# CogSP/CoEvoNet

Measured on AMD Instinct MI355X. Metric: env-steps/sec (agent-steps of the whole job; generations/sec in gens_per_sec), Co-GA simple_adversary_v3 pop=200 HoF=5, higher is better.
Workload: dtype f32

## Files before the change

### coevonet_amd/build.py

```python
import os
import subprocess
import sys
from concurrent.futures import ThreadPoolExecutor

HERE = os.path.dirname(os.path.abspath(__file__))
CSRC = os.path.join(HERE, "csrc")
OBJ = os.path.join(HERE, "csrc", "_obj")
LIB = os.path.join(HERE, "libcoevo.so")
SOURCES = ["fc_forward.hip", "mpe_env.hip", "offspring.hip", "select.hip", "rollout_api.hip", "deepqn.hip",
           "dqn_engine.hip", "host_rollout.hip", "host_placement.hip", "fc16.hip", "fc16_rollout.hip", "fc16_offspring.hip",
           "fc16_es.hip", "dqn16.hip", "dqn16_offspring.hip", "dqn16_es.hip", "dqn16_tiled.hip", "crossplay.hip",
           "sharing.hip"]
FLAGS = ["--offload-arch=gfx950", "-O3", "-std=c++17", "-fPIC", "-ffp-contract=off", "-fno-fast-math", "-Wall",
         "-Wno-unused-function"]


def _headers():
    hs = [os.path.join(CSRC, f) for f in os.listdir(CSRC) if f.endswith(".h")]
    return hs + [os.path.join(HERE, "..", "include", h) for h in ("coevo.h", "coevo_ext.h", "coevo_crossplay.h",
                                                                   "coevo_sharing.h")]


def _stale(target, deps):
    if not os.path.exists(target):
        return True
    t = os.path.getmtime(target)
    return any(os.path.getmtime(d) > t for d in deps)


def _extra_flags():
    return os.environ.get("COEVO_EXTRA_FLAGS", "").split()


def _flag_signature():
    return " ".join(FLAGS + _extra_flags())
# ... 46 lines not shown
```

### coevonet_amd/csrc/mpe_env.hip

```cpp
#include "coevo_common.hip.h"

#include "../../include/coevo_crossplay.h"

namespace coevo {

typedef unsigned __int128 u128;

__host__ __device__ inline u128 pcg_mult()
{
    return (((u128)0x2360ED051FC65DA4ULL) << 64) | (u128)0x4385DF649FCCF645ULL;
}

__host__ __device__ inline uint64_t pcg_output(u128 s)
{
    const uint64_t hi = (uint64_t)(s >> 64), lo = (uint64_t)s;
    const uint64_t x = hi ^ lo;
    const unsigned r = (unsigned)(hi >> 58);
    return (x >> r) | (x << ((64 - r) & 63));
}

__host__ __device__ inline u128 pcg_advance(u128 state, u128 inc, u128 delta)
{
    u128 acc_mult = 1, acc_plus = 0, cur_mult = pcg_mult(), cur_plus = inc;
    while (delta > 0) {
        if (delta & 1) {
            acc_mult *= cur_mult;
            acc_plus = acc_plus * cur_mult + cur_plus;
        }
        cur_plus = (cur_mult + 1) * cur_plus;
        cur_mult *= cur_mult;
        delta >>= 1;
    }
    return acc_mult * state + acc_plus;
}

__host__ __device__ __forceinline__ void mpe_reset_game(double *st, int n, int g, coevo_pcg64 rng, uint64_t ordinal);

__global__ void mpe_reset_kernel(double *st, int n, int game_first, int count, coevo_pcg64 rng,
                                 int64_t first_ordinal, const int32_t *gen_dev, int64_t ordinals_per_gen, int unsigned_first)
{
    const int i = blockIdx.x * blockDim.x + threadIdx.x;
    if (i >= count) return;
    int64_t first = first_ordinal + (gen_dev ? (int64_t)(*gen_dev) * ordinals_per_gen : 0);
    if (first < 0 && !unsigned_first) first = 0;
    mpe_reset_game(st, n, game_first + i, rng, (uint64_t)first + (uint64_t)i);
}

__global__ void mpe_reset_episodes_kernel(double *st, int n, int game_first, int count, coevo_pcg64 rng,
                                          uint64_t first_ordinal, int episodes)
{
    const int i = blockIdx.x * blockDim.x + threadIdx.x;
// ... 5 lines not shown
struct ResetSegs { coevo_reset_seg s[COEVO_MAX_JOBS]; };
__global__ void mpe_reset_multi_kernel(double *st, int n, ResetSegs segs, coevo_pcg64 rng, uint64_t *stamps, int n_stamps,
                                       int32_t *zero_words, int n_zero)
{
    const coevo_reset_seg &sg = segs.s[blockIdx.y];
    const int i = blockIdx.x * blockDim.x + threadIdx.x;
    if (zero_words && blockIdx.y == gridDim.y - 1)
        for (int j = i; j < n_zero; j += gridDim.x * blockDim.x) zero_words[j] = 0;
    if (stamps && blockIdx.y == 0)
        for (int j = i; j < n_stamps; j += gridDim.x * blockDim.x) {
            stamps[2 * j] = ~0ull;
            stamps[2 * j + 1] = 0ull;
        }
    if (i >= sg.count) return;
    mpe_reset_game(st, n, sg.game_first + i, rng, sg.first_ordinal + (uint64_t)i);
}

__host__ __device__ __forceinline__ void mpe_reset_game(double *st, int n, int g, coevo_pcg64 rng, uint64_t ordinal)
{
    const u128 inc = ((u128)rng.pcg_inc_hi << 64) | rng.pcg_inc_lo;
    u128 s = ((u128)rng.pcg_state_hi << 64) | rng.pcg_state_lo;
    s = pcg_advance(s, inc, (u128)(ordinal >> 1) * 21);
    s = s * pcg_mult() + inc;
    const uint64_t c = pcg_output(s);
    const uint32_t half = (ordinal & 1) ? (uint32_t)(c >> 32) : (uint32_t)c;
    const int goal = (int)(((uint64_t)half * 2) >> 32);
    if (ordinal & 1) s = pcg_advance(s, inc, 10);
    double d[10];
#pragma unroll
    for (int i = 0; i < 10; ++i) {
        s = s * pcg_mult() + inc;
        d[i] = -1.0 + 2.0 * ((double)(pcg_output(s) >> 11) * (1.0 / 9007199254740992.0));
    }
    const size_t N = (size_t)n;
#pragma unroll
    for (int i = 0; i < 6; ++i) {
        st[i * N + g] = d[i];
        st[(6 + i) * N + g] = 0.0;
    }
#pragma unroll
    for (int i = 0; i < 4; ++i) st[(12 + i) * N + g] = d[6 + i];
    st[16 * N + g] = d[6 + 2 * goal];
    st[17 * N + g] = d[7 + 2 * goal];
    st[18 * N + g] = 0.0;
    st[19 * N + g] = 0.0;
    st[20 * N + g] = 0.0;
    st[21 * N + g] = 0.0;
    st[22 * N + g] = (double)goal;
    st[23 * N + g] = 0.0;
}

__host__ __device__ inline float mpe_observe_at(const double *st, int n, const int32_t *row_game, const int32_t *row_slot, int i)
{
    const int row = i / COEVO_OBS_STRIDE, k = i % COEVO_OBS_STRIDE;
    const int slot = row_slot[row];
    const int D = (slot == COEVO_SLOT_ADVERSARY) ? 8 : 10;
    return (k < D) ? mpe_obs_element(st, n, row_game[row], slot, k) : 0.0f;
}

__global__ void mpe_observe_kernel(const double *st, int n, const int32_t *row_game, const int32_t *row_slot,
                                   int n_rows, float *obs)
{
    const int i = blockIdx.x * blockDim.x + threadIdx.x;
    if (i >= n_rows * COEVO_OBS_STRIDE) return;
// ... 358 lines not shown
```

### coevonet_amd/csrc/offspring.hip

```cpp
#include "coevo_common.hip.h"
#include "dqn_common.hip.h"
#include "promote_roles.hip.h"
#include "philox.hip.h"

namespace coevo {

__device__ __forceinline__ uint32_t w2_piece_quad(int32_t s0, int32_t o_w2)
{
    const int32_t t = s0 - o_w2;
    const int32_t l = (t >> 2) & 63, kq = (t >> 8) & 127, jb = t >> 15;
    return (uint32_t)((o_w2 + (jb * 64 + l) * H1 + kq * 4) >> 2);
}

__device__ __forceinline__ int32_t w1t_slab_of_flat(uint32_t p, int D)
{
    const uint32_t j = (D == 8) ? (p >> 3) : (p / 10u);
    return (int32_t)((p - j * (uint32_t)D) * H1 + j);
}

__device__ inline void slab_quad_normals(uint64_t seed, uint32_t slo, uint32_t shi, int32_t s0, int D, float z[4])
{
    const int32_t o_b1 = (int32_t)fc_off_b1(D), o_w2 = (int32_t)fc_off_w2(D), o_b2 = (int32_t)fc_off_b2(D);
    const int32_t P = (int32_t)fc_params(D);
    if (s0 >= o_w2 && s0 < o_b2) {
// ... 85 lines not shown
    v = v + dpp_move_f64<0x4E>(v);
    v = v + dpp_move_f64<0x141>(v);
    v = v + dpp_move_f64<0x140>(v);
    v = add_swap_f64<false>(v);
    v = add_swap_f64<true>(v);
    if ((threadIdx.x & 63) == 0) scratch[threadIdx.x >> 6] = v;
    __syncthreads();
    return ((scratch[0] + scratch[1]) + scratch[2]) + scratch[3];
}

#ifndef COEVO_BREED_U
#define COEVO_BREED_U 2
#endif

struct alignas(16) PerturbLds { float z[W1T_MAX_FLOATS]; };

__device__ __forceinline__ void fc_perturb_block(const float *parent_slab, const int32_t *parent_idx, float *child_slab,
                                                 int child_first, int D, const float *sigma_dev, uint64_t seed,
                                                 uint32_t stream_lo_first, uint32_t stream_hi, int skip_layernorm,
                                                 const int32_t *gen_dev, const float *dist_ref, double *dist_partial,
                                                 int c, int bx, int nblocks, PerturbLds &lds)
{
    const int w1t_blocks = D / 2;
    if (bx > 0 && bx < w1t_blocks) return;
    if (gen_dev) stream_hi += 4u * (uint32_t)(*gen_dev);
    const bool antithetic = (skip_layernorm & 2) != 0;
    skip_layernorm &= 1;
    const uint32_t ind = stream_lo_first + (uint32_t)c;
    const uint32_t slo = antithetic ? (ind >> 1) : ind;
    const bool negate = antithetic && (ind & 1u);
// ... 4 lines not shown
    double *scratch = reinterpret_cast<double *>(lds.z);
    if (bx == 0) {
        w1t_normals_to_lds(seed, slo, stream_hi, D, lds.z);
        const float4 *zl = reinterpret_cast<const float4 *>(lds.z);
        float4 zv = zl[threadIdx.x];
        __syncthreads();
        const bool keep[4] = {false, false, false, false}, in_dist[4] = {true, true, true, true};
        for (int b = 0; b < w1t_blocks; ++b) {
            const int32_t s0 = (b * 256 + (int32_t)threadIdx.x) * 4;
            const float4 pv = *reinterpret_cast<const float4 *>(par + s0);
            const float z[4] = {zv.x, zv.y, zv.z, zv.w};
            const double d2 = perturb_apply_piece(pv, z, keep, in_dist, sigma, negate, ch, dist_ref, s0);
            if (b + 1 < w1t_blocks) zv = zl[(b + 1) * 256 + threadIdx.x];
            if (dist_partial) {
                const double tot = breed_block_sum(d2, scratch + 4 * (b & 1));
                if (threadIdx.x == 0) dist_partial[(size_t)c * nblocks + b] = tot;
            }
        }
        return;
    }
#if COEVO_BREED_U > 1
    {
        const int32_t o_w2 = (int32_t)fc_off_w2(D), o_b2 = (int32_t)fc_off_b2(D);
        const int w2_first = (o_w2 + 1023) >> 10, w2_end = o_b2 >> 10;
        if (bx >= w2_first && bx < w2_end) {
            if ((bx - w2_first) % COEVO_BREED_U) return;
            const int run = min(COEVO_BREED_U, w2_end - bx);
            const bool keep[4] = {false, false, false, false}, in_dist[4] = {true, true, true, true};
            double d2u[COEVO_BREED_U];
#pragma unroll
            for (int u = 0; u < COEVO_BREED_U; ++u) {
                d2u[u] = 0.0;
                if (u < run) {
                    const int32_t s0 = ((bx + u) * 256 + (int32_t)threadIdx.x) * 4;
                    const float4 pv = *reinterpret_cast<const float4 *>(par + s0);
                    float z[4];
                    philox_normal4(seed, slo, stream_hi, w2_piece_quad(s0, o_w2), z);
                    d2u[u] = perturb_apply_piece(pv, z, keep, in_dist, sigma, negate, ch, dist_ref, s0);
                }
            }
            if (dist_partial) {
#pragma unroll
                for (int u = 0; u < COEVO_BREED_U; ++u) {
                    if (u < run) {
                        const double tot = breed_block_sum(d2u[u], scratch + 4 * (u & 1));
                        if (threadIdx.x == 0) dist_partial[(size_t)c * nblocks + bx + u] = tot;
                    }
                }
            }
            return;
        }
    }
#endif
    const int32_t s0 = (bx * 256 + (int32_t)threadIdx.x) * 4;
    double d2 = 0.0;
    if (s0 < (int32_t)stride) {
        const float4 pv = *reinterpret_cast<const float4 *>(par + s0);
        float z[4];
        bool keep[4], in_dist[4];
        const int32_t o_w2 = (int32_t)fc_off_w2(D), o_b2 = (int32_t)fc_off_b2(D);
        if (s0 >= o_w2 && s0 < o_b2) {
// ... 3 lines not shown
        } else {
            slab_quad_normals(seed, slo, stream_hi, s0, D, z);
            const int32_t g1 = (int32_t)fc_off_g1(D), g2 = (int32_t)fc_off_g2(D), P = (int32_t)fc_params(D);
            const bool ln = (s0 >= g1 && s0 < g1 + 2 * H1) || (s0 >= g2 && s0 < g2 + 2 * H2);
#pragma unroll
            for (int i = 0; i < 4; ++i) {
                const bool pad = s0 + i >= P;
                keep[i] = pad || (skip_layernorm && ln);
                in_dist[i] = !pad && !ln;
            }
        }
        d2 = perturb_apply_piece(pv, z, keep, in_dist, sigma, negate, ch, dist_ref, s0);
    }
    if (dist_partial) {
        const double tot = breed_block_sum(d2, scratch);
        if (threadIdx.x == 0) dist_partial[(size_t)c * nblocks + bx] = tot;
    }
}

__global__ __launch_bounds__(256) void fc_perturb_kernel(const float *parent_slab, const int32_t *parent_idx,
                                                          float *child_slab, int child_first, int D,
                                                          const float *sigma_dev, uint64_t seed,
                                                          uint32_t stream_lo_first, uint32_t stream_hi,
                                                          int skip_layernorm, const int32_t *gen_dev,
                                                          const float *dist_ref, double *dist_partial)
{
    __shared__ PerturbLds lds;
    fc_perturb_block(parent_slab, parent_idx, child_slab, child_first, D, sigma_dev, seed, stream_lo_first, stream_hi,
                     skip_layernorm, gen_dev, dist_ref, dist_partial, blockIdx.y, blockIdx.x, gridDim.x, lds);
}

static_assert(sizeof(coevo_fc_perturb_job) == 72, "layout mirrored by coevonet_amd/lib.py PerturbJob");
struct PerturbJobs { coevo_fc_perturb_job j[COEVO_MAX_JOBS]; };
__global__ __launch_bounds__(256) void fc_perturb_multi_kernel(PerturbJobs jobs, uint64_t seed, int skip_layernorm,
                                                                const int32_t *gen_dev)
{
    __shared__ PerturbLds lds;
    const coevo_fc_perturb_job &jb = jobs.j[blockIdx.z];
    const int nblocks = (int)quad_blocks(fc_stride(jb.D));
    if ((int)blockIdx.x >= nblocks || (int)blockIdx.y >= jb.n_children) return;
    fc_perturb_block(jb.parent_slab, jb.parent_idx, jb.child_slab, jb.child_first, jb.D, jb.sigma_dev, seed,
                     jb.stream_lo_first, jb.stream_hi, skip_layernorm, gen_dev, jb.dist_ref, jb.dist_partial, blockIdx.y,
                     blockIdx.x, nblocks, lds);
}

__global__ __launch_bounds__(256) void fc_rebuild_elites_kernel(const float *elite_prev, const int32_t *order,
                                                                 float *elite_new, int E, int D,
                                                                 const float *sigma_prev_dev, uint64_t seed,
                                                                 uint32_t stream_hi_prev, const int32_t *gen_dev)
{
    if (gen_dev) stream_hi_prev += 4u * (uint32_t)(*gen_dev - 1);
    const int e = blockIdx.y;
    const int64_t stride = fc_stride(D), P = fc_params(D);
    const int64_t s0 = quad_first(blockIdx.x);
    if (s0 >= stride) return;
    const int id = order[e];
    float *dst = elite_new + (int64_t)e * stride;
    if (id == 0) {
// ... 356 lines not shown
    for (int i = 0; i < n_jobs; ++i) {
        const coevo_fc_perturb_job &j = jobs[i];
        if (!perturb_job_ok(j)) return COEVO_ERR_ARG;
        pj.j[i] = j;
        const unsigned nb = quad_blocks(fc_stride(j.D));
        gx = nb > gx ? nb : gx;
        gy = (unsigned)j.n_children > gy ? (unsigned)j.n_children : gy;
    }
    if (gy == 0) return COEVO_OK;
    hipLaunchKernelGGL(fc_perturb_multi_kernel, dim3(gx, gy, (unsigned)n_jobs), dim3(256), 0, (hipStream_t)stream, pj, seed,
                       skip_layernorm, gen_dev);
    COEVO_HIP_CHECK(hipGetLastError());
    return COEVO_OK;
}

extern "C" int coevo_fc_rebuild_elites(const float *elite_prev, const int32_t *order, float *elite_new, int E, int D,
                                       const float *sigma_prev_dev, uint64_t seed, uint32_t stream_hi_prev,
                                       const int32_t *gen_dev, void *stream)
{
    if (!elite_prev || !order || !elite_new || !sigma_prev_dev || !fc_dim_ok(D) || E <= 0 || E > 65535)
        return COEVO_ERR_ARG;
    if (elite_prev == elite_new) return COEVO_ERR_ARG;
    const dim3 grid(quad_blocks(fc_stride(D)), (unsigned)E);
    hipLaunchKernelGGL(fc_rebuild_elites_kernel, grid, dim3(256), 0, (hipStream_t)stream, elite_prev, order, elite_new,
                       E, D, sigma_prev_dev, seed, stream_hi_prev, gen_dev);
    COEVO_HIP_CHECK(hipGetLastError());
    return COEVO_OK;
}

extern "C" int coevo_net_gather(const float *src_slab, const int32_t *src_idx, float *dst_slab, int dst_first, int n,
// ... 208 lines not shown
```

### coevonet_amd/genetic_algorithm.py

```python
from __future__ import annotations

import os
import time

import numpy as np
import torch

from . import lib as L
from .fcnetwork import FCNetwork
from .ga_half import HalfGAEngine
from .game_logic import create_agent
from .mpe.simple_adversary import ENV_SEED
from .population import (FUSED_MAX_HOF, GA_SHARING_MODES, N_EVAL, RET_SLOT, ROLE_D, ROLES, SIGMA_ATTR, CoGASchedule, CoGATail,
                         NetTable, SlabIO, adapt_mutation_power, captured, co_ga_games, eval_gate_limits, fused_tail_fits,
                         half_route, mean_eval_triple, shard_and_gather, slab_layout)
from .rollout import DeviceRollout, HostEnvRollout, RolloutPlan, effective_steps

ROLE_SLOT = {"agent_0": 1, "agent_1": 2, "adversary_0": 0}


def evaluate_current_weights(agent_0, agent_1, adversary, env, args):
    from .game_logic import play_game
    tot = [0.0, 0.0, 0.0]
    for _ in range(N_EVAL):
        r = play_game(env=env, player1=agent_0.model, player2=agent_1.model, adversary=adversary.model, args=args, eval=True)
        for s in range(3):
            tot[s] += r[s]
    return tot[0] / 10, tot[1] / 10, tot[2] / 10


def mutate_elites(env, elites, args, role):
# ... 163 lines not shown
            self.pair_scratch = torch.zeros(n_scratch, dtype=torch.float64, device=device)
        self.parent_idx = torch.tensor([c % elites for c in range(max(pop - 1, 1))], dtype=torch.int32, device=device)
        self.hof_shift_idx = torch.arange(1, max(hof, 2), dtype=torch.int32, device=device)
        self.iota = torch.arange(max(hof, elites, 2), dtype=torch.int32, device=device)
        self.pblocks = {r: int(L.load().coevo_fc_perturb_blocks(ROLE_D[r])) for r in ROLES}
        self.dist_partial = {r: torch.zeros(max(pop - 1, 1) * self.pblocks[r], dtype=torch.float64, device=device) for r in ROLES}
        self.best_dist = {r: torch.zeros(1, **f32) for r in ROLES}
        one = torch.arange(self.n_local, device=device) * hof + hof - 1
        self._last_game_idx = torch.cat([ph * self.n_local * hof + one for ph in range(3)])
        self.generation = 0
        self.steps_per_generation = 3 * pop * hof * self.T_train + N_EVAL * self.T_eval
        self._dist_current = False
        self._rewards_pin = self._rewards_dev = None
        self._breeding_pending, self.generation_enqueued = False, 0
        self._cohort_streams = self._cohort_done = self._tail_done = self._tail_graph = None
        self.sharded_run, self._sharded_tail_graphs = False, {}
        self.gen_dev = self.sigma64 = self.sigma32 = self.sigma32_prev = self.hist = self.sig_hist = self.loop_args = None
        self.cap, self.fused_tail, self.pipelined, self._gen_graph = 0, False, False, {}

    def _need_device_loop(self):
        if self.gen_dev is None:
            raise RuntimeError("GAEngine: setup_device_loop(args, capacity) has to be called before a device-loop generation")

    def _uploaded(self, region):
        if region in ("pop", "stale"):
            self._dist_current = False
        if region == "hof" and self._hof_tiled:
            self._refresh_hof_twins()

    def _refresh_hof_twins(self):
# ... 193 lines not shown
    def _breed_cohort(self, k, noise_gen, gen_dev=None, tick=False):
        lo_k, hi_k = self._cohort_individuals(k)
        c_lo, c_hi = max(lo_k, 1) - 1, hi_k - 1
        if c_hi > c_lo:
            sigma, stream = self.sigma32.data_ptr(), 0 if gen_dev is not None else noise_gen * 4
            self._breed_children_multi(c_lo, c_hi, (sigma, sigma + 4, sigma + 8), (stream, stream + 1, stream + 2), gen_dev,
                                       L._p(self.gen_dev) if tick else None)
            return
        if lo_k == 0:
            for r in ROLES:
                self.dist[r][0:1].copy_(self.best_dist[r])
        if tick:
            L.call("coevo_counter_add", L._p(self.gen_dev), 1)

    def _reset_cohort(self, k, gen):
        segs = self._reset_segments(gen, *self._cohort_individuals(k), k == self.K - 1 and gen > 0)
        self.ro.reset_segments(segs, arm=(k, self.n_cycles))

    def flush_breeding(self):
        if self._breeding_pending:
            torch.cuda.synchronize()
            for k in range(self.K):
                self._breed_cohort(k, self.generation_enqueued - 1)
            torch.cuda.synchronize()
            self._breeding_pending = False

    def replay_generation_pipelined(self, gen):
        self._need_device_loop()
        assert self.world == 1 and self.env_mode == "device" and self.fused_tail and self.K > 1
        if self.hof_twin is not None and not self._hof_tiled and self.plan.heavy is not None:
            self._enable_hof_tiled()
        self._enqueue_cohort_chains(gen)
# ... 6 lines not shown
    def _enqueue_cohort_chains(self, gen):
        ro = self.ro
        self._gate_evaluation(gen)
        main = torch.cuda.current_stream()
        if self._cohort_streams is None:
            self._cohort_streams = [main] + [
                torch.cuda.ExternalStream(L.load().coevo_rollout_ctx_cohort_stream(ro.ctx, k), device=self.device)
                for k in range(1, self.K)]
            self._cohort_done = [torch.cuda.Event() for _ in range(self.K)]
            self._tail_done = torch.cuda.Event()
        self._tail_done.record(main)
        for k, s in reversed(list(enumerate(self._cohort_streams))):
            if k:
                s.wait_event(self._tail_done)
            with torch.cuda.stream(s):
                if self._breeding_pending:
                    self._breed_cohort(k, gen - 1)
                self._reset_cohort(k, gen)
                ro.enqueue_cohort(k, self.n_cycles, s, armed=True)
            if k:
                self._cohort_done[k].record(s)
        self._breeding_pending = False
        for ev in self._cohort_done[1:]:
            main.wait_event(ev)
        ro.enqueue_final_step(self.n_cycles, pack=self._pack_args() if self._packed_exchange() else None)

    def _packed_exchange(self):
        return (self.sharded_run and self.fused_tail and self.gather_packed is not None
                and os.environ.get("COEVO_PACKED_EXCHANGE", "1") != "0")

    def _pack_args(self):
        return (self.pack_local, self.dist_all, 3, self.n_local, self.hof, self.pop, self.lo)

# ... 330 lines not shown
```

### coevonet_amd/lib.py

```python
from __future__ import annotations

import ctypes as C
import math
import os
import re

import numpy as np
import torch

HERE = os.path.dirname(os.path.abspath(__file__))
LIB_PATH = os.environ.get("COEVO_LIB") or os.path.join(HERE, "libcoevo.so")
HEADER_PATH = os.path.join(HERE, "..", "include", "coevo.h")
EXT_HEADER_PATH = os.path.join(HERE, "..", "include", "coevo_ext.h")
CROSSPLAY_HEADER_PATH = os.path.join(HERE, "..", "include", "coevo_crossplay.h")
SHARING_HEADER_PATH = os.path.join(HERE, "..", "include", "coevo_sharing.h")


class CoevoError(RuntimeError):
    pass


_SCALARS = {"int": C.c_int, "int32_t": C.c_int32, "int64_t": C.c_int64, "uint32_t": C.c_uint32, "uint64_t": C.c_uint64,
            "size_t": C.c_size_t, "float": C.c_float, "double": C.c_double}
_POINTED_TO = ("void", "char", "uint8_t")


def _declare(text, structs, decl, spec=None):
    m = re.fullmatch(r"([\w\s]*?)\s*(\**)\s*(\w+)\s*(?:\[(\d+)\])?", text.strip())
    words = [w for w in (m.group(1).split() if m else []) if w not in ("const", "struct")]
    if not m or len(words) > 1 or not (words or spec):
# ... 103 lines not shown

K_XP, _XP_SIGS = _parse_crossplay_header(_header_text(CROSSPLAY_HEADER_PATH))


def _parse_sharing_header(text):
    consts, structs, sigs = parse_header(text, known=STRUCTS)
    if (set(structs) != set(STRUCTS) or set(sigs) & (set(_SIGS) | set(_EXT_SIGS) | set(_XP_SIGS))
            or set(consts) & (set(K) | set(K_EXT) | set(K_XP))):
        raise CoevoError("include/coevo_sharing.h: declares a struct or repeats a name of include/coevo.h, include/coevo_ext.h "
                         "or include/coevo_crossplay.h")
    return consts, sigs


K_SH, _SH_SIGS = _parse_sharing_header(_header_text(SHARING_HEADER_PATH))

OBS_STRIDE, LOGIT_STRIDE, FC_MAX_ROWS = K["COEVO_OBS_STRIDE"], K["COEVO_LOGIT_STRIDE"], K["COEVO_FC_MAX_ROWS"]
MPE_STATE_DOUBLES, STAMP_SLOTS = K["COEVO_MPE_STATE_DOUBLES"], K["COEVO_STAMP_SLOTS"]
ST_NAMES = {K["COEVO_ST_BAD_INPUT"]: "input contains inf or NaN",
            K["COEVO_ST_BAD_FC1"]: "output contains inf or NaN after fc1",
            K["COEVO_ST_BAD_FC2"]: "output contains inf or NaN after fc2",
            K["COEVO_ST_BAD_OUT"]: "output contains inf or NaN",
            K["COEVO_ST_NO_ACTION"]: "no action selected (current_best_position = -1)",
            K["COEVO_ST_SYNC_TIMEOUT"]: "persistent rollout: a workgroup timed out waiting for the other rows of its games "
                                        "(COEVO_ST_SYNC_TIMEOUT)",
            K["COEVO_ST_BAD_TASK"]: "fp16 forward: a task with a bad width, row count or unaligned net offset was skipped "
                                    "(COEVO_ST_BAD_TASK)"}

DQN_LOGIT_STRIDE, DQN_MAX_ROWS = K["COEVO_DQN_LOGIT_STRIDE"], K["COEVO_DQN_MAX_ROWS"]
DQN_FC1_TILED = K["COEVO_DQN_FC1_TILED"]
DQP_SKIP_BN = K["COEVO_DQP_SKIP_BN"]
# ... 31 lines not shown
    return sorted(_SIGS)


def extension_symbols():
    return sorted(_EXT_SIGS)


def crossplay_symbols():
    return sorted(_XP_SIGS)


def sharing_symbols():
    return sorted(_SH_SIGS)


def load():
    global _lib
    if _lib is None:
        if not os.path.exists(LIB_PATH):
            raise CoevoError(f"{LIB_PATH} is missing: build the HIP extension first "
                             "(python -m coevonet_amd.build); there is no CPU fallback")
        L = C.CDLL(LIB_PATH)
        for name, (res, args) in {**_SIGS, **_EXT_SIGS, **_XP_SIGS, **_SH_SIGS}.items():
            fn = getattr(L, name)
            fn.restype = res
            fn.argtypes = args
        flags = (L.coevo_build_flags() or b"").decode()
        if flags and os.environ.get("COEVO_ALLOW_VARIANT") != "1":
            raise CoevoError(f"{LIB_PATH} was built with non-default switches ({flags}): a measurement variant, not the "
                             "product (rebuild with python -m coevonet_amd.build, or set COEVO_ALLOW_VARIANT=1 in tools/)")
        _lib = L
    return _lib


def _check(rc, what):
    if rc != 0:
        raise CoevoError(f"{what} failed with code {rc} "
                         f"({'bad argument' if rc == -1 else 'HIP runtime error' if rc == -2 else 'unsupported here' if rc == -3 else 'unknown'})")
# ... 70 lines not shown
```

### coevonet_amd/population.py

```python
from __future__ import annotations

import ctypes as ct
import os

import numpy as np
import torch

from . import lib as L
from .rollout import DeviceRollout, RolloutPlan

ROLES = ("agent_0", "agent_1", "adversary_0")
ROLE_D = {"agent_0": 10, "agent_1": 10, "adversary_0": 8}
RET_SLOT = {"agent_0": 0, "agent_1": 1, "adversary_0": 2}
ROLES2 = ("first_0", "second_0")
N_EVAL = 10
ES_CHUNKS = 8
SIGMA_ATTR = {"agent_0": "mutation_power_agent_0", "agent_1": "mutation_power_agent_1",
              "adversary_0": "mutation_power_adversary"}


def slab_layout(roles, regions, stride_of):
    base, off = {}, 0
    for r in roles:
        base[r] = {}
# ... 300 lines not shown

    def _promote_unfused(self, r, best_to_pop0=True, best_dist=False):
        self._hof_push(r)
        if best_to_pop0:
            self._best_to_pop0(r)
        if best_dist:
            L.call("coevo_gather_f32", L._p(self.best_dist[r]), L._p(self.dist[r]), L._p(self.order[r]), 1)

    def _breed_role_children(self, ri, r, c_lo, c_hi, stream, gen_dev, sigma_ptr):
        L.call(self._perturb_dist_entry, self._ptr(r, "elite"), self.parent_idx.data_ptr() + 4 * c_lo, self._ptr(r, "pop"),
               1 + c_lo, c_hi - c_lo, ROLE_D[r], sigma_ptr, self.philox_seed, c_lo, stream, 0, gen_dev, self._ptr(r, "stale"),
               L._p(self.dist_partial[r]))
        L.call(self._finalize_entry, L._p(self.dist_partial[r]), self.pblocks[r], c_hi - c_lo, L._p(self.dist[r]), 1 + c_lo,
               L._p(self.best_dist[r]) if c_lo == 0 else None)

    def _breed_children_multi(self, c_lo, c_hi, sigma_ptrs, streams, gen_dev=None, tick=None):
        Job = getattr(L, self._perturb_job)
        pj, fj = (Job * 3)(), (L.FinalizeJob * 3)()
        for ri, r in enumerate(ROLES):
            part = self.dist_partial[r].data_ptr() + 8 * c_lo * self.pblocks[r]
            pj[ri] = Job(self._ptr(r, "elite"), self.parent_idx.data_ptr() + 4 * c_lo, self._ptr(r, "pop"), sigma_ptrs[ri],
                         self._ptr(r, "stale"), part, 1 + c_lo, c_hi - c_lo, ROLE_D[r], c_lo, streams[ri], 0)
            fj[ri] = L.FinalizeJob(part, self.dist[r].data_ptr(), self.best_dist[r].data_ptr() if c_lo == 0 else None,
                                   self.pblocks[r], c_hi - c_lo, 1 + c_lo, 0)
        L.call(self._perturb_multi_entry, ct.cast(pj, ct.c_void_p), 3, self.philox_seed, 0, gen_dev)
        if tick is not None:
            L.call(self._finalize_multi_entry + "_tick", ct.cast(fj, ct.c_void_p), 3, tick)
        else:
            L.call(self._finalize_multi_entry, ct.cast(fj, ct.c_void_p), 3)


class CoESSchedule:

    def _rollout_pair(self, games, eval_games, table, env_seed, cls=DeviceRollout, host_cohorts=None, **ro_kw):
        cohorts = int(os.environ.get("COEVO_ES_COHORTS", "2")) if host_cohorts is None else host_cohorts
        game_cohort = None
        if host_cohorts is not None and cohorts > 1 and len(games) >= cohorts:
            game_cohort = (np.arange(len(games)) * cohorts // len(games)).astype(np.int32)
        self.plan = RolloutPlan(np.array(games), table.net_off, table.net_D, device=self.device,
# ... 169 lines not shown
```

### coevonet_amd/rollout.py

```python
from __future__ import annotations

import ctypes as _ct

import os

import numpy as np
import torch

from . import lib as L
from .mpe import simple_adversary as sa

LIGHT_ROWS = 8
HEAVY_ROWS = 32


class RolloutPlan:

    def __init__(self, game_nets, net_off, net_D, device="cuda", heavy_rows=HEAVY_ROWS, n_cohorts=1,
                 game_cohort=None, split_rows=None, row_order="class", resident_nets=()):
        game_nets = np.asarray(game_nets, dtype=np.int64)
        self.n_games = int(game_nets.shape[0])
        by_net = {}
        for g in range(self.n_games):
            for slot in range(3):
# ... 122 lines not shown

    def cohort_tasks(self, k):
        out = ()
        for tasks, tnp, begin in ((self.heavy, self.heavy_np, self.heavy_begin_np), (self.light, self.light_np, self.light_begin_np)):
            b, e = int(begin[k]), int(begin[k + 1])
            ptr = tasks.data_ptr() + b * L.TASK_DTYPE.itemsize if (tasks is not None and e > b) else None
            out += (ptr, e - b, int(max(tnp["n_rows"][b:e], default=0)))
        return out

    def distinct_weight_bytes_per_cycle(self):
        seen = {}
        for arr in (self.heavy_np, self.light_np):
            for t in arr:
                seen[int(t["net_off"])] = L.fc_param_count(int(t["D"])) * 4
        return sum(seen.values())


def effective_steps(limit, max_cycles):
    cap = 3 * max_cycles
    return cap if limit is None else min(int(limit), cap)


def last_buffer(n_cycles):
    last = int(n_cycles) - 1
    return last & 1 if last > 0 else 0


class DeviceRollout:

    def __init__(self, plan: RolloutPlan, slab: torch.Tensor, env_seed=sa.ENV_SEED, timing_pairs=0, fused_step=True,
# ... 65 lines not shown
        try:
            if getattr(self, "ctx", None):
                L.load().coevo_rollout_ctx_destroy(self.ctx)
                self.ctx = None
        except Exception:
            pass

    def set_limits(self, limits_np):
        self.limits.copy_(torch.from_numpy(np.asarray(limits_np, dtype=np.int32)), non_blocking=False)

    def reset(self, game_first, n_games, first_ordinal):
        L.call("coevo_mpe_reset", L._p(self.state), self.plan.n_games, int(game_first), int(n_games), self.rng,
               int(first_ordinal))

    def reset_segments(self, segs, arm=None):
        arr = (L.ResetSeg * len(segs))(*[L.ResetSeg(int(a), int(b), int(c)) for a, b, c in segs])
        if arm is not None:
            k, n_cycles = arm
            n_cycles = int(n_cycles)
            if k is not None and not 0 <= int(k) < self.n_cohorts:
                raise ValueError(f"arm: cohort {k} of a rollout with {self.n_cohorts}")
            if not 0 < n_cycles <= self.stamp_cycles:
                raise ValueError(f"arm: {n_cycles} cycles (1 .. {self.stamp_cycles})")
            first, count = (0, self.n_cohorts) if k is None else (int(k), 1)
            stamps, sync = self._cohort_scratch(first, n_cycles)
            if stamps or sync:
                L.call("coevo_mpe_reset_multi_prep", L._p(self.state), self.plan.n_games, _ct.cast(arr, _ct.c_void_p), len(segs),
                       self.rng, stamps, count * n_cycles * L.STAMP_SLOTS if stamps else 0, sync,
                       count * self.sync_words_per_cohort if sync else 0)
            else:
                L.call("coevo_mpe_reset_multi", L._p(self.state), self.plan.n_games, _ct.cast(arr, _ct.c_void_p), len(segs),
                       self.rng)
            for c in range(first, first + count):
                self._armed[c] = (n_cycles, bool(self.time_light))
            return
        L.call("coevo_mpe_reset_multi", L._p(self.state), self.plan.n_games, _ct.cast(arr, _ct.c_void_p), len(segs), self.rng)

    def _take_arm(self, cohorts, n_cycles, armed):
        if armed:
            for c in cohorts:
                if self._armed.get(c) != (int(n_cycles), bool(self.time_light)):
                    raise ValueError(f"armed=True, but cohort {c} was not armed for {n_cycles} cycles"
                                     f"{' with timed stamps' if self.time_light else ''} by reset_segments(arm=...) since its "
                                     f"last rollout (armed: {self._armed})")
        for c in cohorts:
            self._armed.pop(c, None)

    def _cohort_scratch(self, k, n_cycles):
        stamps = (self.stamps.data_ptr() + 16 * L.STAMP_SLOTS * int(k) * int(n_cycles)) if self.time_light else None
        sync = (self.sync_words.data_ptr() + 4 * int(k) * self.sync_words_per_cohort) if self.sync_words is not None else None
        return stamps, sync
# ... 262 lines not shown
```

Before: 153.8 million.

## Fuse per-cohort breeding, distance finalize and env reset into one turnover kernel

Adds a ga_turnover_kernel that, in a single launch, runs the per-cohort episode resets, stamp and sync-word clears, the perturbation of the children and their distance partials. The last workgroup for each child is detected with an atomic ticket counter and reduces the distance partials in place. In the pipelined Co-GA loop, the separate perturb, finalize and reset launches per cohort are replaced by this one call, which cuts launch count and host overhead per cohort. In exchange it uses atomic ticket counters with relaxed ordering and a waitcnt, so correctness depends on memory visibility between workgroups, and the reset blocks now share a grid with the heavier perturb blocks.

```diff
diff --git a/coevonet_amd/build.py b/coevonet_amd/build.py
--- a/coevonet_amd/build.py
+++ b/coevonet_amd/build.py
@@ -18,7 +18,7 @@
 def _headers():
     hs = [os.path.join(CSRC, f) for f in os.listdir(CSRC) if f.endswith(".h")]
     return hs + [os.path.join(HERE, "..", "include", h) for h in ("coevo.h", "coevo_ext.h", "coevo_crossplay.h",
-                                                                   "coevo_sharing.h")]
+                                                                   "coevo_sharing.h", "coevo_turnover.h")]
 
 
 def _stale(target, deps):
diff --git a/coevonet_amd/csrc/mpe_env.hip b/coevonet_amd/csrc/mpe_env.hip
--- a/coevonet_amd/csrc/mpe_env.hip
+++ b/coevonet_amd/csrc/mpe_env.hip
@@ -1,40 +1,10 @@
 #include "coevo_common.hip.h"
+#include "mpe_reset.hip.h"
 
 #include "../../include/coevo_crossplay.h"
 
 namespace coevo {
 
-typedef unsigned __int128 u128;
-
-__host__ __device__ inline u128 pcg_mult()
-{
-    return (((u128)0x2360ED051FC65DA4ULL) << 64) | (u128)0x4385DF649FCCF645ULL;
-}
-
-__host__ __device__ inline uint64_t pcg_output(u128 s)
-{
-    const uint64_t hi = (uint64_t)(s >> 64), lo = (uint64_t)s;
-    const uint64_t x = hi ^ lo;
-    const unsigned r = (unsigned)(hi >> 58);
-    return (x >> r) | (x << ((64 - r) & 63));
-}
-
-__host__ __device__ inline u128 pcg_advance(u128 state, u128 inc, u128 delta)
-{
-    u128 acc_mult = 1, acc_plus = 0, cur_mult = pcg_mult(), cur_plus = inc;
-    while (delta > 0) {
-        if (delta & 1) {
-            acc_mult *= cur_mult;
-            acc_plus = acc_plus * cur_mult + cur_plus;
-        }
-        cur_plus = (cur_mult + 1) * cur_plus;
-        cur_mult *= cur_mult;
-        delta >>= 1;
-    }
-    return acc_mult * state + acc_plus;
-}
-
-__host__ __device__ __forceinline__ void mpe_reset_game(double *st, int n, int g, coevo_pcg64 rng, uint64_t ordinal);
 
 __global__ void mpe_reset_kernel(double *st, int n, int game_first, int count, coevo_pcg64 rng,
                                  int64_t first_ordinal, const int32_t *gen_dev, int64_t ordinals_per_gen, int unsigned_first)
@@ -70,40 +40,6 @@
         }
     if (i >= sg.count) return;
     mpe_reset_game(st, n, sg.game_first + i, rng, sg.first_ordinal + (uint64_t)i);
-}
-
-__host__ __device__ __forceinline__ void mpe_reset_game(double *st, int n, int g, coevo_pcg64 rng, uint64_t ordinal)
-{
-    const u128 inc = ((u128)rng.pcg_inc_hi << 64) | rng.pcg_inc_lo;
-    u128 s = ((u128)rng.pcg_state_hi << 64) | rng.pcg_state_lo;
-    s = pcg_advance(s, inc, (u128)(ordinal >> 1) * 21);
-    s = s * pcg_mult() + inc;
-    const uint64_t c = pcg_output(s);
-    const uint32_t half = (ordinal & 1) ? (uint32_t)(c >> 32) : (uint32_t)c;
-    const int goal = (int)(((uint64_t)half * 2) >> 32);
-    if (ordinal & 1) s = pcg_advance(s, inc, 10);
-    double d[10];
-#pragma unroll
-    for (int i = 0; i < 10; ++i) {
-        s = s * pcg_mult() + inc;
-        d[i] = -1.0 + 2.0 * ((double)(pcg_output(s) >> 11) * (1.0 / 9007199254740992.0));
-    }
-    const size_t N = (size_t)n;
-#pragma unroll
-    for (int i = 0; i < 6; ++i) {
-        st[i * N + g] = d[i];
-        st[(6 + i) * N + g] = 0.0;
-    }
-#pragma unroll
-    for (int i = 0; i < 4; ++i) st[(12 + i) * N + g] = d[6 + i];
-    st[16 * N + g] = d[6 + 2 * goal];
-    st[17 * N + g] = d[7 + 2 * goal];
-    st[18 * N + g] = 0.0;
-    st[19 * N + g] = 0.0;
-    st[20 * N + g] = 0.0;
-    st[21 * N + g] = 0.0;
-    st[22 * N + g] = (double)goal;
-    st[23 * N + g] = 0.0;
 }
 
 __host__ __device__ inline float mpe_observe_at(const double *st, int n, const int32_t *row_game, const int32_t *row_slot, int i)
diff --git a/coevonet_amd/csrc/mpe_reset.hip.h b/coevonet_amd/csrc/mpe_reset.hip.h
--- /dev/null
+++ b/coevonet_amd/csrc/mpe_reset.hip.h
@@ -0,0 +1,70 @@
+#pragma once
+#include "coevo_common.hip.h"
+
+namespace coevo {
+
+typedef unsigned __int128 u128;
+
+__host__ __device__ inline u128 pcg_mult()
+{
+    return (((u128)0x2360ED051FC65DA4ULL) << 64) | (u128)0x4385DF649FCCF645ULL;
+}
+
+__host__ __device__ inline uint64_t pcg_output(u128 s)
+{
+    const uint64_t hi = (uint64_t)(s >> 64), lo = (uint64_t)s;
+    const uint64_t x = hi ^ lo;
+    const unsigned r = (unsigned)(hi >> 58);
+    return (x >> r) | (x << ((64 - r) & 63));
+}
+
+__host__ __device__ inline u128 pcg_advance(u128 state, u128 inc, u128 delta)
+{
+    u128 acc_mult = 1, acc_plus = 0, cur_mult = pcg_mult(), cur_plus = inc;
+    while (delta > 0) {
+        if (delta & 1) {
+            acc_mult *= cur_mult;
+            acc_plus = acc_plus * cur_mult + cur_plus;
+        }
+        cur_plus = (cur_mult + 1) * cur_plus;
+        cur_mult *= cur_mult;
+        delta >>= 1;
+    }
+    return acc_mult * state + acc_plus;
+}
+
+__host__ __device__ __forceinline__ void mpe_reset_game(double *st, int n, int g, coevo_pcg64 rng, uint64_t ordinal)
+{
+    const u128 inc = ((u128)rng.pcg_inc_hi << 64) | rng.pcg_inc_lo;
+    u128 s = ((u128)rng.pcg_state_hi << 64) | rng.pcg_state_lo;
+    s = pcg_advance(s, inc, (u128)(ordinal >> 1) * 21);
+    s = s * pcg_mult() + inc;
+    const uint64_t c = pcg_output(s);
+    const uint32_t half = (ordinal & 1) ? (uint32_t)(c >> 32) : (uint32_t)c;
+    const int goal = (int)(((uint64_t)half * 2) >> 32);
+    if (ordinal & 1) s = pcg_advance(s, inc, 10);
+    double d[10];
+#pragma unroll
+    for (int i = 0; i < 10; ++i) {
+        s = s * pcg_mult() + inc;
+        d[i] = -1.0 + 2.0 * ((double)(pcg_output(s) >> 11) * (1.0 / 9007199254740992.0));
+    }
+    const size_t N = (size_t)n;
+#pragma unroll
+    for (int i = 0; i < 6; ++i) {
+        st[i * N + g] = d[i];
+        st[(6 + i) * N + g] = 0.0;
+    }
+#pragma unroll
+    for (int i = 0; i < 4; ++i) st[(12 + i) * N + g] = d[6 + i];
+    st[16 * N + g] = d[6 + 2 * goal];
+    st[17 * N + g] = d[7 + 2 * goal];
+    st[18 * N + g] = 0.0;
+    st[19 * N + g] = 0.0;
+    st[20 * N + g] = 0.0;
+    st[21 * N + g] = 0.0;
+    st[22 * N + g] = (double)goal;
+    st[23 * N + g] = 0.0;
+}
+
+}
diff --git a/coevonet_amd/csrc/offspring.hip b/coevonet_amd/csrc/offspring.hip
--- a/coevonet_amd/csrc/offspring.hip
+++ b/coevonet_amd/csrc/offspring.hip
@@ -2,6 +2,9 @@
 #include "dqn_common.hip.h"
 #include "promote_roles.hip.h"
 #include "philox.hip.h"
+#include "mpe_reset.hip.h"
+
+#include "../../include/coevo_turnover.h"
 
 namespace coevo {
 
@@ -123,6 +126,11 @@
 #endif
 
 struct alignas(16) PerturbLds { float z[W1T_MAX_FLOATS]; };
+
+__device__ __forceinline__ void store_partial(double *p, double v)
+{
+    __hip_atomic_store(p, v, __ATOMIC_RELAXED, __HIP_MEMORY_SCOPE_AGENT);
+}
 
 __device__ __forceinline__ void fc_perturb_block(const float *parent_slab, const int32_t *parent_idx, float *child_slab,
                                                  int child_first, int D, const float *sigma_dev, uint64_t seed,
@@ -157,7 +165,7 @@
             if (b + 1 < w1t_blocks) zv = zl[(b + 1) * 256 + threadIdx.x];
             if (dist_partial) {
                 const double tot = breed_block_sum(d2, scratch + 4 * (b & 1));
-                if (threadIdx.x == 0) dist_partial[(size_t)c * nblocks + b] = tot;
+                if (threadIdx.x == 0) store_partial(dist_partial + (size_t)c * nblocks + b, tot);
             }
         }
         return;
@@ -187,7 +195,7 @@
                 for (int u = 0; u < COEVO_BREED_U; ++u) {
                     if (u < run) {
                         const double tot = breed_block_sum(d2u[u], scratch + 4 * (u & 1));
-                        if (threadIdx.x == 0) dist_partial[(size_t)c * nblocks + bx + u] = tot;
+                        if (threadIdx.x == 0) store_partial(dist_partial + (size_t)c * nblocks + bx + u, tot);
                     }
                 }
             }
@@ -221,7 +229,7 @@
     }
     if (dist_partial) {
         const double tot = breed_block_sum(d2, scratch);
-        if (threadIdx.x == 0) dist_partial[(size_t)c * nblocks + bx] = tot;
+        if (threadIdx.x == 0) store_partial(dist_partial + (size_t)c * nblocks + bx, tot);
     }
 }
 
@@ -249,6 +257,65 @@
     fc_perturb_block(jb.parent_slab, jb.parent_idx, jb.child_slab, jb.child_first, jb.D, jb.sigma_dev, seed,
                      jb.stream_lo_first, jb.stream_hi, skip_layernorm, gen_dev, jb.dist_ref, jb.dist_partial, blockIdx.y,
                      blockIdx.x, nblocks, lds);
+}
+
+struct TurnoverJobs {
+    coevo_fc_perturb_job p[COEVO_MAX_JOBS];
+    coevo_fc_finalize_job f[COEVO_MAX_JOBS];
+    coevo_reset_seg s[COEVO_MAX_JOBS];
+};
+struct TurnoverGrid { uint32_t reset_wgs, rx, n_segs, gx, gy; };
+
+__global__ __launch_bounds__(256) void ga_turnover_kernel(TurnoverJobs tj, TurnoverGrid gd, uint64_t seed, int skip_layernorm,
+                                                          const int32_t *gen_dev, uint32_t *tickets, double *st, int n,
+                                                          coevo_pcg64 rng, uint64_t *stamps, int n_stamps, int32_t *zero_words,
+                                                          int n_zero)
+{
+    __shared__ PerturbLds lds;
+    uint32_t wg = blockIdx.x;
+    if (wg < gd.reset_wgs) {
+        const uint32_t sy = wg / gd.rx;
+        const int i = (int)((wg % gd.rx) * 256u + threadIdx.x), span = (int)(gd.rx * 256u);
+        if (zero_words && sy == gd.n_segs - 1)
+            for (int j = i; j < n_zero; j += span) zero_words[j] = 0;
+        if (stamps && sy == 0)
+            for (int j = i; j < n_stamps; j += span) {
+                stamps[2 * j] = ~0ull;
+                stamps[2 * j + 1] = 0ull;
+            }
+        const coevo_reset_seg &sg = tj.s[sy];
+        if (i < sg.count) mpe_reset_game(st, n, sg.game_first + i, rng, sg.first_ordinal + (uint64_t)i);
+        return;
+    }
+    wg -= gd.reset_wgs;
+    const uint32_t bx = wg % gd.gx, cy = wg / gd.gx, c = cy % gd.gy, job = cy / gd.gy;
+    const coevo_fc_perturb_job &jb = tj.p[job];
+    const int nblocks = (int)quad_blocks(fc_stride(jb.D));
+    if ((int)bx >= nblocks || (int)c >= jb.n_children) return;
+    fc_perturb_block(jb.parent_slab, jb.parent_idx, jb.child_slab, jb.child_first, jb.D, jb.sigma_dev, seed,
+                     jb.stream_lo_first, jb.stream_hi, skip_layernorm, gen_dev, jb.dist_ref, jb.dist_partial, (int)c, (int)bx,
+                     nblocks, lds);
+    __syncthreads();
+    int *last = reinterpret_cast<int *>(lds.z) + 16;
+    if (threadIdx.x == 0) {
+        uint32_t *t = tickets + (size_t)job * gd.gy + c;
+        __builtin_amdgcn_s_waitcnt(0);
+        const uint32_t before = __hip_atomic_fetch_add(t, 1u, __ATOMIC_RELAXED, __HIP_MEMORY_SCOPE_AGENT);
+        *last = before == (uint32_t)nblocks - 1u;
+        if (*last) __hip_atomic_store(t, 0u, __ATOMIC_RELAXED, __HIP_MEMORY_SCOPE_AGENT);
+    }
+    __syncthreads();
+    if (!*last || threadIdx.x >= 64) return;
+    const coevo_fc_finalize_job &fj = tj.f[job];
+    const double *pp = fj.dist_partial + (size_t)c * fj.n_blocks;
+    double v = 0.0;
+    for (int b = threadIdx.x; b < fj.n_blocks; b += 64) v += __hip_atomic_load(pp + b, __ATOMIC_RELAXED, __HIP_MEMORY_SCOPE_AGENT);
+#pragma unroll
+    for (int m = 1; m < 64; m <<= 1) v = v + __shfl_xor(v, m, 64);
+    if (threadIdx.x == 0) {
+        fj.dist[fj.first + (int)c] = (float)sqrt(v);
+        if (c == 0 && fj.head) fj.dist[fj.first - 1] = *fj.head;
+    }
 }
 
 __global__ __launch_bounds__(256) void fc_rebuild_elites_kernel(const float *elite_prev, const int32_t *order,
@@ -635,6 +702,50 @@
     return COEVO_OK;
 }
 
+extern "C" int coevo_ga_turnover(const coevo_fc_perturb_job *jobs, const coevo_fc_finalize_job *fin, int n_jobs, uint64_t seed,
+                                 int skip_layernorm, const int32_t *gen_dev, uint32_t *tickets, double *state, int n_games,
+                                 const coevo_reset_seg *segs, int n_segs, coevo_pcg64 rng, uint64_t *stamps, int n_stamps,
+                                 int32_t *zero_words, int n_zero, void *stream)
+{
+    if (!jobs || !fin || !tickets || n_jobs < 1 || n_jobs > COEVO_MAX_JOBS || skip_layernorm < 0 || skip_layernorm > 3)
+        return COEVO_ERR_ARG;
+    if (!state || n_games <= 0 || !segs || n_segs < 1 || n_segs > COEVO_MAX_JOBS) return COEVO_ERR_ARG;
+    if ((stamps && n_stamps <= 0) || (zero_words && n_zero <= 0)) return COEVO_ERR_ARG;
+    TurnoverJobs tj{};
+    uint32_t gx = 0, gy = 0;
+    for (int i = 0; i < n_jobs; ++i) {
+        const coevo_fc_perturb_job &j = jobs[i];
+        const coevo_fc_finalize_job &f = fin[i];
+        if (!perturb_job_ok(j) || !j.dist_partial) return COEVO_ERR_ARG;
+        const uint32_t nb = quad_blocks(fc_stride(j.D));
+        if (f.dist_partial != j.dist_partial || !f.dist || f.n_blocks != (int)nb || f.n != j.n_children || f.first < 0 ||
+            (f.head && f.first < 1))
+            return COEVO_ERR_ARG;
+        tj.p[i] = j;
+        tj.f[i] = f;
+        gx = nb > gx ? nb : gx;
+        gy = (uint32_t)j.n_children > gy ? (uint32_t)j.n_children : gy;
+    }
+    int cmax = 0;
+    for (int i = 0; i < n_segs; ++i) {
+        if (segs[i].game_first < 0 || segs[i].count < 0 || segs[i].game_first + segs[i].count > n_games) return COEVO_ERR_ARG;
+        tj.s[i] = segs[i];
+        cmax = segs[i].count > cmax ? segs[i].count : cmax;
+    }
+    if (!stamps) n_stamps = 0;
+    if (!zero_words) n_zero = 0;
+    const bool resets = cmax > 0 || stamps || zero_words;
+    const uint32_t rx = cmax > 0 ? (uint32_t)(cmax + 255) / 256u : 1u;
+    const TurnoverGrid gd{resets ? rx * (uint32_t)n_segs : 0u, rx, (uint32_t)n_segs, gx, gy};
+    const uint64_t total = (uint64_t)gd.reset_wgs + (uint64_t)gx * gy * (uint32_t)n_jobs;
+    if (total == 0) return COEVO_OK;
+    if (total > 0xffffffffull) return COEVO_ERR_ARG;
+    hipLaunchKernelGGL(ga_turnover_kernel, dim3((uint32_t)total), dim3(256), 0, (hipStream_t)stream, tj, gd, seed, skip_layernorm,
+                       gen_dev, tickets, state, n_games, rng, stamps, n_stamps, zero_words, n_zero);
+    COEVO_HIP_CHECK(hipGetLastError());
+    return COEVO_OK;
+}
+
 extern "C" int coevo_fc_rebuild_elites(const float *elite_prev, const int32_t *order, float *elite_new, int E, int D,
                                        const float *sigma_prev_dev, uint64_t seed, uint32_t stream_hi_prev,
                                        const int32_t *gen_dev, void *stream)
diff --git a/coevonet_amd/genetic_algorithm.py b/coevonet_amd/genetic_algorithm.py
--- a/coevonet_amd/genetic_algorithm.py
+++ b/coevonet_amd/genetic_algorithm.py
@@ -1,5 +1,6 @@
 from __future__ import annotations
 
+import ctypes as ct
 import os
 import time
 
@@ -14,7 +15,7 @@
 from .population import (FUSED_MAX_HOF, GA_SHARING_MODES, N_EVAL, RET_SLOT, ROLE_D, ROLES, SIGMA_ATTR, CoGASchedule, CoGATail,
                          NetTable, SlabIO, adapt_mutation_power, captured, co_ga_games, eval_gate_limits, fused_tail_fits,
                          half_route, mean_eval_triple, shard_and_gather, slab_layout)
-from .rollout import DeviceRollout, HostEnvRollout, RolloutPlan, effective_steps
+from .rollout import DeviceRollout, HostEnvRollout, RolloutPlan, effective_steps, reset_seg_array
 
 ROLE_SLOT = {"agent_0": 1, "agent_1": 2, "adversary_0": 0}
 
@@ -208,6 +209,7 @@
         self._rewards_pin = self._rewards_dev = None
         self._breeding_pending, self.generation_enqueued = False, 0
         self._cohort_streams = self._cohort_done = self._tail_done = self._tail_graph = None
+        self._turnover_tickets = None
         self.sharded_run, self._sharded_tail_graphs = False, {}
         self.gen_dev = self.sigma64 = self.sigma32 = self.sigma32_prev = self.hist = self.sig_hist = self.loop_args = None
         self.cap, self.fused_tail, self.pipelined, self._gen_graph = 0, False, False, {}
@@ -431,8 +433,34 @@
             L.call("coevo_counter_add", L._p(self.gen_dev), 1)
 
     def _reset_cohort(self, k, gen):
-        segs = self._reset_segments(gen, *self._cohort_individuals(k), k == self.K - 1 and gen > 0)
-        self.ro.reset_segments(segs, arm=(k, self.n_cycles))
+        self.ro.reset_segments(self._cohort_segments(k, gen), arm=(k, self.n_cycles))
+
+    def _cohort_segments(self, k, gen):
+        return self._reset_segments(gen, *self._cohort_individuals(k), k == self.K - 1 and gen > 0)
+
+    def _turnover_args(self, k, gen):
+        lo_k, hi_k = self._cohort_individuals(k)
+        c_lo, c_hi = max(lo_k, 1) - 1, hi_k - 1
+        if c_hi <= c_lo:
+            return None
+        sigma, stream = self.sigma32.data_ptr(), (gen - 1) * 4
+        pj, fj = self._multi_jobs(c_lo, c_hi, (sigma, sigma + 4, sigma + 8), (stream, stream + 1, stream + 2))
+        return pj, fj, self._cohort_segments(k, gen)
+
+    def _turnover_cohort(self, k, gen):
+        args = self._turnover_args(k, gen) if self._breeding_pending else None
+        if args is None:
+            if self._breeding_pending:
+                self._breed_cohort(k, gen - 1)
+            self._reset_cohort(k, gen)
+            return
+        pj, fj, segs = args
+        if self._turnover_tickets is None:
+            self._turnover_tickets = torch.zeros(self.K, 3 * max(self.pop, 1), dtype=torch.int32, device=self.device)
+        ro, arr = self.ro, reset_seg_array(segs)
+        L.call("coevo_ga_turnover", ct.cast(pj, ct.c_void_p), ct.cast(fj, ct.c_void_p), 3, self.philox_seed, 0, None,
+               self._turnover_tickets[k].data_ptr(), L._p(ro.state), self.plan.n_games, ct.cast(arr, ct.c_void_p), len(segs),
+               ro.rng, *ro.arm_scratch(k, self.n_cycles))
 
     def flush_breeding(self):
         if self._breeding_pending:
@@ -469,9 +497,7 @@
             if k:
                 s.wait_event(self._tail_done)
             with torch.cuda.stream(s):
-                if self._breeding_pending:
-                    self._breed_cohort(k, gen - 1)
-                self._reset_cohort(k, gen)
+                self._turnover_cohort(k, gen)
                 ro.enqueue_cohort(k, self.n_cycles, s, armed=True)
             if k:
                 self._cohort_done[k].record(s)
diff --git a/coevonet_amd/lib.py b/coevonet_amd/lib.py
--- a/coevonet_amd/lib.py
+++ b/coevonet_amd/lib.py
@@ -14,6 +14,7 @@
 EXT_HEADER_PATH = os.path.join(HERE, "..", "include", "coevo_ext.h")
 CROSSPLAY_HEADER_PATH = os.path.join(HERE, "..", "include", "coevo_crossplay.h")
 SHARING_HEADER_PATH = os.path.join(HERE, "..", "include", "coevo_sharing.h")
+TURNOVER_HEADER_PATH = os.path.join(HERE, "..", "include", "coevo_turnover.h")
 
 
 class CoevoError(RuntimeError):
@@ -147,6 +148,17 @@
 
 K_SH, _SH_SIGS = _parse_sharing_header(_header_text(SHARING_HEADER_PATH))
 
+
+def _parse_turnover_header(text):
+    consts, structs, sigs = parse_header(text, known=STRUCTS)
+    if (set(structs) != set(STRUCTS) or set(sigs) & (set(_SIGS) | set(_EXT_SIGS) | set(_XP_SIGS) | set(_SH_SIGS))
+            or set(consts) & (set(K) | set(K_EXT) | set(K_XP) | set(K_SH))):
+        raise CoevoError("include/coevo_turnover.h: declares a struct or repeats a name of another header")
+    return consts, sigs
+
+
+K_TO, _TO_SIGS = _parse_turnover_header(_header_text(TURNOVER_HEADER_PATH))
+
 OBS_STRIDE, LOGIT_STRIDE, FC_MAX_ROWS = K["COEVO_OBS_STRIDE"], K["COEVO_LOGIT_STRIDE"], K["COEVO_FC_MAX_ROWS"]
 MPE_STATE_DOUBLES, STAMP_SLOTS = K["COEVO_MPE_STATE_DOUBLES"], K["COEVO_STAMP_SLOTS"]
 ST_NAMES = {K["COEVO_ST_BAD_INPUT"]: "input contains inf or NaN",
@@ -208,6 +220,10 @@
     return sorted(_SH_SIGS)
 
 
+def turnover_symbols():
+    return sorted(_TO_SIGS)
+
+
 def load():
     global _lib
     if _lib is None:
@@ -215,7 +231,7 @@
             raise CoevoError(f"{LIB_PATH} is missing: build the HIP extension first "
                              "(python -m coevonet_amd.build); there is no CPU fallback")
         L = C.CDLL(LIB_PATH)
-        for name, (res, args) in {**_SIGS, **_EXT_SIGS, **_XP_SIGS, **_SH_SIGS}.items():
+        for name, (res, args) in {**_SIGS, **_EXT_SIGS, **_XP_SIGS, **_SH_SIGS, **_TO_SIGS}.items():
             fn = getattr(L, name)
             fn.restype = res
             fn.argtypes = args
diff --git a/coevonet_amd/population.py b/coevonet_amd/population.py
--- a/coevonet_amd/population.py
+++ b/coevonet_amd/population.py
@@ -338,7 +338,7 @@
         L.call(self._finalize_entry, L._p(self.dist_partial[r]), self.pblocks[r], c_hi - c_lo, L._p(self.dist[r]), 1 + c_lo,
                L._p(self.best_dist[r]) if c_lo == 0 else None)
 
-    def _breed_children_multi(self, c_lo, c_hi, sigma_ptrs, streams, gen_dev=None, tick=None):
+    def _multi_jobs(self, c_lo, c_hi, sigma_ptrs, streams):
         Job = getattr(L, self._perturb_job)
         pj, fj = (Job * 3)(), (L.FinalizeJob * 3)()
         for ri, r in enumerate(ROLES):
@@ -347,6 +347,10 @@
                          self._ptr(r, "stale"), part, 1 + c_lo, c_hi - c_lo, ROLE_D[r], c_lo, streams[ri], 0)
             fj[ri] = L.FinalizeJob(part, self.dist[r].data_ptr(), self.best_dist[r].data_ptr() if c_lo == 0 else None,
                                    self.pblocks[r], c_hi - c_lo, 1 + c_lo, 0)
+        return pj, fj
+
+    def _breed_children_multi(self, c_lo, c_hi, sigma_ptrs, streams, gen_dev=None, tick=None):
+        pj, fj = self._multi_jobs(c_lo, c_hi, sigma_ptrs, streams)
         L.call(self._perturb_multi_entry, ct.cast(pj, ct.c_void_p), 3, self.philox_seed, 0, gen_dev)
         if tick is not None:
             L.call(self._finalize_multi_entry + "_tick", ct.cast(fj, ct.c_void_p), 3, tick)
diff --git a/coevonet_amd/rollout.py b/coevonet_amd/rollout.py
--- a/coevonet_amd/rollout.py
+++ b/coevonet_amd/rollout.py
@@ -160,6 +160,10 @@
             for t in arr:
                 seen[int(t["net_off"])] = L.fc_param_count(int(t["D"])) * 4
         return sum(seen.values())
+
+
+def reset_seg_array(segs):
+    return (L.ResetSeg * len(segs))(*[L.ResetSeg(int(a), int(b), int(c)) for a, b, c in segs])
 
 
 def effective_steps(limit, max_cycles):
@@ -255,27 +259,30 @@
                int(first_ordinal))
 
     def reset_segments(self, segs, arm=None):
-        arr = (L.ResetSeg * len(segs))(*[L.ResetSeg(int(a), int(b), int(c)) for a, b, c in segs])
+        arr = reset_seg_array(segs)
         if arm is not None:
-            k, n_cycles = arm
-            n_cycles = int(n_cycles)
-            if k is not None and not 0 <= int(k) < self.n_cohorts:
-                raise ValueError(f"arm: cohort {k} of a rollout with {self.n_cohorts}")
-            if not 0 < n_cycles <= self.stamp_cycles:
-                raise ValueError(f"arm: {n_cycles} cycles (1 .. {self.stamp_cycles})")
-            first, count = (0, self.n_cohorts) if k is None else (int(k), 1)
-            stamps, sync = self._cohort_scratch(first, n_cycles)
+            stamps, n_stamps, sync, n_sync = self.arm_scratch(*arm)
             if stamps or sync:
                 L.call("coevo_mpe_reset_multi_prep", L._p(self.state), self.plan.n_games, _ct.cast(arr, _ct.c_void_p), len(segs),
-                       self.rng, stamps, count * n_cycles * L.STAMP_SLOTS if stamps else 0, sync,
-                       count * self.sync_words_per_cohort if sync else 0)
+                       self.rng, stamps, n_stamps, sync, n_sync)
             else:
                 L.call("coevo_mpe_reset_multi", L._p(self.state), self.plan.n_games, _ct.cast(arr, _ct.c_void_p), len(segs),
                        self.rng)
-            for c in range(first, first + count):
-                self._armed[c] = (n_cycles, bool(self.time_light))
             return
         L.call("coevo_mpe_reset_multi", L._p(self.state), self.plan.n_games, _ct.cast(arr, _ct.c_void_p), len(segs), self.rng)
+
+    def arm_scratch(self, k, n_cycles):
+        n_cycles = int(n_cycles)
+        if k is not None and not 0 <= int(k) < self.n_cohorts:
+            raise ValueError(f"arm: cohort {k} of a rollout with {self.n_cohorts}")
+        if not 0 < n_cycles <= self.stamp_cycles:
+            raise ValueError(f"arm: {n_cycles} cycles (1 .. {self.stamp_cycles})")
+        first, count = (0, self.n_cohorts) if k is None else (int(k), 1)
+        stamps, sync = self._cohort_scratch(first, n_cycles)
+        for c in range(first, first + count):
+            self._armed[c] = (n_cycles, bool(self.time_light))
+        return (stamps, count * n_cycles * L.STAMP_SLOTS if stamps else 0, sync,
+                count * self.sync_words_per_cohort if sync else 0)
 
     def _take_arm(self, cohorts, n_cycles, armed):
         if armed:
diff --git a/include/coevo_turnover.h b/include/coevo_turnover.h
--- /dev/null
+++ b/include/coevo_turnover.h
@@ -0,0 +1,17 @@
+#ifndef COEVO_TURNOVER_H
+#define COEVO_TURNOVER_H
+#include "coevo.h"
+
+#ifdef __cplusplus
+extern "C" {
+#endif
+
+int coevo_ga_turnover(const coevo_fc_perturb_job *jobs , const coevo_fc_finalize_job *fin , int n_jobs,
+                      uint64_t seed, int skip_layernorm, const int32_t *gen_dev, uint32_t *tickets, double *state, int n_games,
+                      const coevo_reset_seg *segs , int n_segs, coevo_pcg64 rng, uint64_t *stamps, int n_stamps,
+                      int32_t *zero_words, int n_zero, void *stream);
+
+#ifdef __cplusplus
+}
+#endif
+#endif
```

Result: slower. 146.6 million (-4.7%).
